# nirajbabar/raytracinginonesemester

Hardware: AMD Instinct MI355X
Metric: Mrays/s at 1920x1080x16spp (1/2/4/8 GPU) + PPM max-abs pixel diff (higher is better)
Workload: dtype f32+f64

## Files before the change

include/rt_mi355x.h:

```cpp
#ifndef RT_MI355X_H
#define RT_MI355X_H

#include <stddef.h>
#include <stdint.h>

#ifdef __cplusplus
extern "C" {
#endif

#define RT_ABI_VERSION 3

enum {
    RT_OK = 0,
    RT_ERR_ARG = -1,
    RT_ERR_IO = -2,
    RT_ERR_PARSE = -3,
    RT_ERR_HIP = -4,
    RT_ERR_NOMEM = -5,
    RT_ERR_NODEVICE = -6,
    RT_ERR_UNSUPPORTED = -7,
    RT_ERR_COMM = -8,
    RT_ERR_INTERNAL = -9
};

// ... 408 lines not shown
int rt_heavy_tiles(const rt_scene* s, int64_t* heavy);
const char* rt_scene_kernel_name(const rt_scene* s);

int rt_scene_traversal_info(const rt_scene* s, int64_t info[4]);
int rt_scene_faults(rt_scene* s, uint32_t* flags, int clear);

typedef enum {
    RT_TUNE_FRUSTUM_ARITY = 0,
    RT_TUNE_HALF_WAVES = 1,
    RT_TUNE_PAIRED_ONLY = 2,
    RT_TUNE_HEAVY_FRAC = 3,
    RT_TUNE_HEAVY_CAP = 4,
    RT_TUNE_CULL_COVERAGE = 5,
    RT_TUNE_CULL_BOXES = 6,
    RT_TUNE_BIG_SCENE_BYTES = 7,
    RT_TUNE_FRUSTUM_STACK_CAP = 8,
    RT_TUNE_PEER_TIMEOUT_S = 9,
    RT_TUNE_RENDERER_THREADS = 10,
    RT_TUNE_COPY_ENGINE = 11,
    RT_TUNE_QUANT_RECORDS = 12,
    RT_TUNE_PREPASS_GATE = 13,
    RT_TUNE_OVERLAP_FRAMES = 14,
    RT_TUNE_KERNEL_TIMING_EVERY = 15,
    RT_TUNE_RECORD_GREEDY = 16,
    RT_TUNE_WIDE4_GREEDY = 17,
    RT_TUNE_PAIR_FRAMES = 18,
    RT_TUNE_PAIR_RESERVE = 19,
    RT_TUNE_CUT_SUB = 20,
    RT_TUNE_HW1_LANES = 21,
    RT_TUNE_COPY_WAIT = 22,
    RT_TUNE_HW1_FUSE = 23,
    RT_TUNE_HW1_CHUNK = 24,
    RT_TUNE_FRAME_STREAMS = 25,
    RT_TUNE_COUNT = 26
} rt_tune_id;
int rt_tuning_set(int id, double value);
int rt_tuning_get(int id, double* value);
void rt_tuning_reset(void);

int rt_device_count(int* n);
const char* rt_last_error(void);
int rt_abi_version(void);
const char* rt_build_id(void);

#ifdef __cplusplus
}
#endif
#endif
```

raytracinginonesemester_amd/_lib.py:

```python
from __future__ import annotations

import ctypes as C
import os
from pathlib import Path

PKG = Path(__file__).resolve().parent
LIB_PATH = Path(os.environ.get("RT_MI355X_LIB", PKG / "lib" / "librt_mi355x.so"))

RT_OK = 0
RT_ERR = {
    -1: "RT_ERR_ARG", -2: "RT_ERR_IO", -3: "RT_ERR_PARSE", -4: "RT_ERR_HIP",
    -5: "RT_ERR_NOMEM", -6: "RT_ERR_NODEVICE", -7: "RT_ERR_UNSUPPORTED", -8: "RT_ERR_COMM",
    -9: "RT_ERR_INTERNAL",
}
RT_KERNEL_AUTO, RT_KERNEL_WAVE, RT_KERNEL_LANE, RT_KERNEL_WAVE_PIXELS = 0, 1, 2, 3
RT_TILES_AUTO, RT_TILES_LINEAR, RT_TILES_XCD_CHUNK, RT_TILES_ROWS = 0, 1, 2, 3
RT_FLAG_NO_CULL = 1
RT_FLAG_BINARY = 4
RT_DELIVER_P6, RT_DELIVER_F32, RT_DELIVER_DEVICE, RT_DELIVER_NONE = 0, 1, 2, 3
RT_GATHER_AUTO, RT_GATHER_RCCL, RT_GATHER_DIRECT, RT_GATHER_HOST_SHARED = 0, 1, 2, 3
RT_RENDERER_SELF_SEND = 1
RT_TIME_GATHER, RT_TIME_DELIVER, RT_TIME_FRAME = 0, 1, 2
RT_FAULT_FRUSTUM_STACK = 1
RT_RAYS_CLOSEST, RT_RAYS_OCCLUDED = 0, 1
RT_RAYS_VARIANT_NONE, RT_RAYS_VARIANT_WIDE, RT_RAYS_VARIANT_BINARY, RT_RAYS_VARIANT_DEEP = 0, 1, 2, 3
RT_REBUILD_NONE, RT_REBUILD_DEVICE, RT_REBUILD_HOST = 0, 1, 2
RT_PATH_LAST = 16
RT_PATH_NONE = 0xFFFFFFFF
RT_PIXEL_NONE = 0xFFFFFFFF
TUNE = {"frustum_arity": 0, "half_waves": 1, "paired_only": 2, "heavy_frac": 3, "heavy_cap": 4,
        "cull_coverage": 5, "cull_boxes": 6, "big_scene_bytes": 7, "frustum_stack_cap": 8,
        "peer_timeout_s": 9, "renderer_threads": 10, "copy_engine": 11,
        "quant_records": 12, "prepass_gate": 13,
        "overlap_frames": 14, "kernel_timing_every": 15,
        "record_greedy": 16, "wide4_greedy": 17, "pair_frames": 18, "pair_reserve": 19,
        "cut_sub": 20, "hw1_lanes": 21, "copy_wait": 22, "hw1_fuse": 23, "hw1_chunk": 24,
        "frame_streams": 25}


class RTError(RuntimeError):
    def __init__(self, code: int, msg: str):
        super().__init__(f"{RT_ERR.get(code, code)}: {msg}")
        self.code = code


class Vec3(C.Structure):
    _fields_ = [("x", C.c_float), ("y", C.c_float), ("z", C.c_float)]

    def __iter__(self):
        return iter((self.x, self.y, self.z))


class BVHNode(C.Structure):
    _fields_ = [("parent_idx", C.c_uint32), ("left_idx", C.c_uint32),
                ("right_idx", C.c_uint32), ("object_idx", C.c_uint32)]


class AABB(C.Structure):
    _fields_ = [("min_corner", Vec3), ("max_corner", Vec3)]


class Triangle(C.Structure):
    _fields_ = [("v0", Vec3), ("v1", Vec3), ("v2", Vec3), ("n0", Vec3), ("n1", Vec3), ("n2", Vec3)]


class Material(C.Structure):
    _fields_ = [("albedo", Vec3), ("kd", C.c_float), ("specular_color", Vec3), ("ks", C.c_float),
                ("shininess", C.c_float), ("kr", C.c_float), ("emission", Vec3)]


# ... 257 lines not shown
```

raytracinginonesemester_amd/csrc/rt_device.hip:

```cpp

#include <hip/hip_runtime.h>
#include <hip/hip_ext.h>

#include <cfloat>
#include <cmath>
#include <cstdint>
#include <cstdio>
#include <cstdlib>
#include <cstring>
#include <algorithm>
#include <atomic>
#include <functional>
#include <memory>
#include <new>
#include <string>
#include <array>
#include <vector>

#include "rt_common.hpp"
#include "rt_hip_host.hpp"
#include "rt_math.hpp"
#include "rt_ppm.hpp"
#include "rt_scene_pack.hpp"

using namespace rtd;

namespace {

using rt::LEAF_BIT;
using rt::NO_REF;
using rt::FRUSTUM_STACK;
using rt::STACK_CAP;
using rt::LANE_LDS_CAP;
using rt::kBigSceneBytes;
constexpr uint32_t RT_FAULT_FRUSTUM_STACK = 1u;
constexpr uint32_t VER_FORCE = 0xFFFFFFFFu;
constexpr int BLOCK = 256;
constexpr int MODE_WIDE = 16;
constexpr int MODE_PK = 32;
constexpr int MODE_DEEP = 64;
constexpr int MODE_1L = 128;
constexpr int MODE_QR = 256;
constexpr int REF_STACK = 512;
constexpr uint32_t INV_LEAF = 0xFFFFFFFEu;
constexpr uint32_t BRUTE_BIT = 0x40000000u;
constexpr float RT_EPS = 1e-3f;

struct DevMaterial {
    float albedo[3], kd, spec[3], ks, shininess, kr, emission[3];
};
struct DevLight {
    float pos[3], color[3];
    int32_t intensity;
};

struct SceneView {
    const float4* __restrict__ inode;
    const float4* __restrict__ wnode;
    const float* __restrict__ fnode;
    int32_t f_log2;
    const uint4* __restrict__ qent;
    const float4* __restrict__ qhdr;
    const float4* __restrict__ ibox;
    const float4* __restrict__ rootb;
    const float4* __restrict__ leaf;
    const float4* __restrict__ tnorm;
    const int32_t* __restrict__ objids;
    const DevMaterial* __restrict__ mats;
    const DevLight* __restrict__ lights;
    int32_t num_tris, num_mats, num_lights;
    uint32_t root_ref;
    float root_box[6];
    float bmax[3];
    int32_t wide;
    int32_t lane_stack;
    int32_t lane_wide;
    const float* __restrict__ cut;
    int32_t ncut;
    const float* __restrict__ cut2;
    int32_t cut_sub_log2;
    const float4* __restrict__ tri;
    uint32_t* fault;
};

__device__ __forceinline__ f3 scene_bmax(const SceneView& sc) { return mk(sc.bmax[0], sc.bmax[1], sc.bmax[2]); }

struct RenderParams {
    SceneView sc;
    f3 cam_center, cam_p00, cam_du, cam_dv;
    int32_t W, H, spp, max_depth, diffuse_bounce;
    f3 miss;
    const float* __restrict__ jitter;
    int32_t band_rows, band_index, band_count, rows;
    int32_t tile_w, tile_h, tiles_x, tiles_total;
    int32_t lane_samples;
    int32_t half_waves;
    int32_t paired_only;
    int32_t tile_order;
    int32_t spp_log2, tile_w_log2;
    int32_t cull;
    f3 miss_pixel;
    uint32_t* live_count;
    int32_t* live_tiles;
    int32_t* cut_tiles;
    uint32_t* next_count;
    int32_t cut_force;
    int32_t nqueues;
    int32_t queue_cap;
    float* __restrict__ rgb;
    int32_t* __restrict__ hit_idx;
    float* __restrict__ hit_t;
    uint8_t* __restrict__ p6;
    uint8_t miss_p6[4];
    uint16_t* __restrict__ tile_cost;
    int32_t* heavy_tiles;
    int32_t heavy_cap;
    uint32_t heavy_ticks[8];
    unsigned long long* ray_count;
    uint32_t* drained;
    uint32_t drain_tag;
    int32_t gate_q8;
};

#include "rt_wave.hpp"
#include "rt_instrument.hpp"
#include "rt_traverse.hpp"
#include "rt_shade.hpp"
#include "rt_prepass.hpp"
#include "rt_query.hpp"
#include "rt_path.hpp"
#include "rt_refit.hpp"
#include "rt_rebuild.hpp"

__device__ __forceinline__ int work_length(const RenderParams& P, int q, int& heavy) {
    heavy = 0;
    if (P.heavy_cap > 0)
        for (int k = 0; k < NCLASS; ++k) heavy += min((int)ldc_u32(P.live_count + heavy_counter(k, q)), P.heavy_cap);
    const int slot = P.sc.ncut > 0 ? CUT_SLOT0 + q : q;
    return heavy + (int)ldc_u32(&P.live_count[slot * COUNTER_STRIDE]);
}

// ... 1234 lines not shown
    hipExtLaunchKernelGGL(KERNEL, grid, dim3(BLOCK), 0, L.st, L.start, L.stop, 0, P);
}

template <int MODE, bool SAMPLES, bool D1, int WAVES = RT_RENDER_WAVES, int LS = 0>
void launch_render_pair(const RenderParams& A, const RenderParams& B, const Launch& L, double reserve_default) {
    constexpr auto KERNEL = render_pair_kernel<MODE, SAMPLES, D1, WAVES, LS>;
    static const int per_cu = [] {
        int n = 0;
        if (hipOccupancyMaxActiveBlocksPerMultiprocessor(&n, KERNEL, BLOCK, 0) != hipSuccess || n < 1) n = 1;
        return n;
    }();
    static const std::string name = "render_pair_kernel<" + std::to_string(MODE) + (SAMPLES ? ", true" : ", false") +
                                    (D1 ? ", true, " : ", false, ") + std::to_string(WAVES) + ", " +
                                    std::to_string(LS) + ">";
    if (L.name) *L.name = name.c_str();
    const int tiles8 = (A.tiles_total + B.tiles_total + 7) / 8 * 8;
    const double reserve = std::clamp(rt::tuning(RT_TUNE_PAIR_RESERVE, reserve_default), 0.0, double(per_cu - 1));
    const int blocks = L.cus * per_cu - int(std::lround(reserve * L.cus));
    const dim3 grid((unsigned)std::max(8, std::min(tiles8, blocks / 8 * 8)));
    PairParams PP;
    PP.f[0] = A;
    PP.f[1] = B;
    hipExtLaunchKernelGGL(KERNEL, grid, dim3(BLOCK), 0, L.st, L.start, L.stop, 0, PP);
}

bool pair_kernel_fits(const RenderParams& P, bool samples, bool wave_wide, bool big) {
    const bool d1 = P.max_depth == 1;
    const bool bounce = P.max_depth > 1 && P.half_waves && P.paired_only;
    return samples && wave_wide && !big && (d1 || bounce) && P.nqueues == 8 && P.spp <= 64 && !P.ray_count &&
           P.lane_samples == 1;
}
void launch_pair(const RenderParams& A, const RenderParams& B, const Launch& L) {
    constexpr int M = RT_KERNEL_WAVE | MODE_WIDE | MODE_PK;
    if (A.max_depth > 1) launch_render_pair<RT_KERNEL_WAVE | MODE_WIDE, true, false, RT_PAIRED_WAVES, 3>(A, B, L, 0.0);
    else if (A.half_waves) launch_render_pair<M, true, true, RT_RENDER_WAVES, 1>(A, B, L, 1.0);
    else launch_render_pair<M, true, true>(A, B, L, 1.0);
}

template <int MODE, bool SAMPLES>
void launch_mode(const RenderParams& P, const Launch& L) {
    constexpr int D1_MODE = (MODE & (MODE_DEEP | RT_KERNEL_LANE)) == 0 ? (MODE | MODE_PK) : MODE;
    if (P.max_depth == 1) {
        if constexpr (SAMPLES) {
            if (P.half_waves) {
                launch_render<D1_MODE, SAMPLES, true, RT_RENDER_WAVES, 1>(P, L);
                return;
            }
        }
        if constexpr ((MODE & (MODE_DEEP | RT_KERNEL_LANE)) == 0) {
            if (L.big) {
                if constexpr ((MODE & MODE_WIDE) != 0) {
                    if (L.qr) {
                        if (P.sc.num_lights == 1)
                            launch_render<D1_MODE | MODE_1L | MODE_QR, SAMPLES, true, RT_RENDER_WAVES_BIG>(P, L);
                        else launch_render<D1_MODE | MODE_QR, SAMPLES, true, RT_RENDER_WAVES_BIG>(P, L);
                        return;
                    }
                }
                if (P.sc.num_lights == 1) launch_render<D1_MODE | MODE_1L, SAMPLES, true, RT_RENDER_WAVES_BIG>(P, L);
                else launch_render<D1_MODE, SAMPLES, true, RT_RENDER_WAVES_BIG>(P, L);
                return;
            }
        }
        launch_render<D1_MODE, SAMPLES, true>(P, L);
    } else {
        if constexpr (SAMPLES && (MODE & (MODE_DEEP | RT_KERNEL_LANE)) == 0) {
            if (P.half_waves && P.paired_only) {
                launch_render<MODE, SAMPLES, false, RT_PAIRED_WAVES, 3>(P, L);
                return;
            }
        }
        if constexpr (SAMPLES) {
            if (P.half_waves) {
                launch_render<MODE, SAMPLES, false, RT_BOUNCE_WAVES, 1>(P, L);
                return;
            }
        }
        launch_render<MODE, SAMPLES, false, RT_BOUNCE_WAVES>(P, L);
    }
}

template <int MODE>
void launch(const RenderParams& P, bool samples, const Launch& L) {
    if (samples) launch_mode<MODE, true>(P, L);
    else launch_mode<MODE, false>(P, L);
}

f3 miss_pixel_value(const rt_render_opts* o) {
    f3 c = mk(0.f, 0.f, 0.f);
    if (o->max_depth > 0)
        c = clamp01(add(mk(0.f, 0.f, 0.f), mul(mk(1.f, 1.f, 1.f), f3{o->miss_color.x, o->miss_color.y, o->miss_color.z})));
    f3 acc = mk(0.f, 0.f, 0.f);
    for (int k = 0; k < o->spp; ++k) acc = add(acc, c);
    const float fs = (float)o->spp;
    return f3{acc.x / fs, acc.y / fs, acc.z / fs};
}

// ... 139 lines not shown
    P.hit_idx = hit_idx;
    P.hit_t = hit_t;
    P.p6 = p6;
    P.ray_count = t_ray_count;
    {
        const f3 mp = miss_pixel_value(o);
        P.miss_p6[0] = rtp::p6_default_sample(mp.x);
        P.miss_p6[1] = rtp::p6_default_sample(mp.y);
        P.miss_p6[2] = rtp::p6_default_sample(mp.z);
        P.miss_p6[3] = 0;
    }
    const bool samples = o->kernel != RT_KERNEL_WAVE_PIXELS && o->spp <= BLOCK && (o->spp & (o->spp - 1)) == 0;
    int half = o->band_count >= 4 || o->max_depth > 1 ? 1 : 0;
    if (const double h = rt::tuning(RT_TUNE_HALF_WAVES, -1.0); h >= 0.0) half = h >= 1.0 ? 1 : 0;
    if (!samples || o->spp > (64 >> half)) half = 0;
    P.half_waves = half;
    P.paired_only = half && o->max_depth > 1 && s->nlights == 1 && !s->deep && o->kernel != RT_KERNEL_LANE &&
                            (P.sc.wide ? s->lane_wide : s->lane_stack)
                        ? 1
                        : 0;
    P.paired_only = P.paired_only && rt::tuning(RT_TUNE_PAIRED_ONLY, 1.0) != 0.0;
    int ppb = samples ? (BLOCK >> half) / o->spp : BLOCK;
    int tw = 1;
    while (tw * tw < ppb) tw <<= 1;
    int th = ppb / tw;
    P.tile_w = tw;
    P.tile_h = th;
    P.tile_w_log2 = __builtin_ctz(unsigned(tw));
    P.spp_log2 = samples ? __builtin_ctz(unsigned(o->spp)) : 0;
    P.tiles_x = (W + tw - 1) / tw;
    const int tiles_y = (rows + th - 1) / th;
    P.tiles_total = P.tiles_x * tiles_y;
    P.lane_samples = samples ? 1 : 0;
    P.tile_order = o->tile_order == RT_TILES_AUTO ? RT_TILES_ROWS : o->tile_order;
    P.cull = (o->flags & RT_FLAG_NO_CULL) ? 0 : 1;
    if (!P.cull) P.sc.ncut = 0;
    P.miss_pixel = miss_pixel_value(o);
    P.nqueues = P.tile_order == RT_TILES_LINEAR ? 1 : 8;
    P.queue_cap = P.tile_order == RT_TILES_LINEAR ? P.tiles_total : P.tiles_x * ((tiles_y + 7) / 8);
    const double heavy_frac = rt::tuning(RT_TUNE_HEAVY_FRAC, 0.10);
    const int mode = o->kernel == RT_KERNEL_LANE ? RT_KERNEL_LANE : RT_KERNEL_WAVE;
    const bool costs = P.cull && P.sc.ncut > 0 && P.nqueues == 8 && heavy_frac > 0.0;
    const int heavy_cap = int(std::clamp(rt::tuning(RT_TUNE_HEAVY_CAP, 512.0), 1.0, 1e9));
    P.heavy_cap = costs ? std::min(P.queue_cap, heavy_cap) : 0;
    constexpr size_t kCounterBytes = COUNTER_SET_U32 * sizeof(uint32_t);
    const size_t list_bytes = size_t(P.nqueues) * size_t(P.queue_cap) * sizeof(int32_t);
    const size_t cut_bytes = P.sc.ncut > 0 ? list_bytes : 0;
    const size_t heavy_bytes = size_t(8 * NCLASS) * size_t(P.heavy_cap) * sizeof(int32_t);
    const size_t set_bytes = list_bytes + cut_bytes + heavy_bytes;
    const size_t work_bytes = rt_scene::kSets * (kCounterBytes + set_bytes);
    hipStream_t st = static_cast<hipStream_t>(stream);
    const uint64_t k = s->launches;
    auto ev1_of = [&](uint64_t f) { return s->ev1[f % rt_scene::kRing]; };
    bool pair_b = ps && ps->phase == 1 && ps->deferred;
    if (pair_b) {
        const RenderParams& A = ps->A;
        const bool same = A.tiles_total == P.tiles_total && A.tiles_x == P.tiles_x && A.W == P.W && A.rows == P.rows &&
                          A.spp == P.spp && A.half_waves == P.half_waves && A.sc.ncut == P.sc.ncut && A.cull == P.cull &&
                          A.heavy_cap == P.heavy_cap && A.queue_cap == P.queue_cap && A.nqueues == P.nqueues &&
                          A.max_depth == P.max_depth && A.paired_only == P.paired_only && A.band_index == P.band_index &&
                          A.band_count == P.band_count && ps->stream == static_cast<hipStream_t>(stream);
        if (!same) {
            pair_b = false;
            if ((rc = flush_pair_a(s, *ps)) != RT_OK) return rc;
        }
    }
// ... 1086 lines not shown
```

raytracinginonesemester_amd/csrc/rt_shade.hpp:

```cpp
#pragma once

template <bool DEEP = false>
__device__ __forceinline__ int32_t leaf_tri(const SceneView& sc, int32_t slot) {
    if constexpr (DEEP) {
        if ((uint32_t)slot & BRUTE_BIT) return (int32_t)((uint32_t)slot & ~BRUTE_BIT);
    }
    return __float_as_int(sc.leaf[4 * (size_t)slot].w);
}

struct SurfHit {
    f3 p, n;
    int32_t tri;
};

template <bool DEEP = false>
__device__ __forceinline__ SurfHit resolve_hit(const SceneView& sc, const RayPre& r, int32_t slot) {
    const float4* L = sc.leaf + 4 * (size_t)slot;
    bool brute = false;
    if constexpr (DEEP) {
        brute = ((uint32_t)slot & BRUTE_BIT) != 0;
        if (brute) L = sc.tri + 3 * (size_t)((uint32_t)slot & ~BRUTE_BIT);
    }
    const float4 a = L[0], b = L[1], c = L[2];
    const f3 v0 = mk(a.x, a.y, a.z), e1 = mk(b.x, b.y, b.z), e2 = mk(b.w, c.x, c.y);
// ... 88 lines not shown
            const SurfHit sh = resolve_hit<(MODE & MODE_DEEP) != 0>(sc, cray, slot);
            const f3 N = unit(sh.n);
            const f3 V = unit(sub(cray.o, sh.p));
            const f3 L = unit(sub(lpos, sh.p));
            const float NdotL = fmaxf(dot(N, L), 0.0f);
            if (NdotL > 0.0f) {
                const DevMaterial m = material_of(sc, sh.tri);
                const f3 f = eval_brdf(m, sh.n, V, L);
                const f3 rad = scale(mk(lt.color[0], lt.color[1], lt.color[2]), (float)lt.intensity);
                Lo_lit = add(Lo, scale(mul(rad, f), NdotL));
                lit = true;
                const f3 toL = sub(lpos, sh.p);
                dist = sqrtf(dot(toL, toL));
                if (dist > 0.0f) {
                    need = true;
                    sray = make_ray(add(sh.p, scale(N, RT_EPS)), divf(toL, dist), scene_bmax(sc));
                }
            }
        }
        pk.put(0, cray.d.x);
        pk.put(1, cray.d.y);
        pk.put(2, cray.d.z);
        pk.put(3, __int_as_float(slot));
        pk.put(4, Lo.x);
        pk.put(5, Lo.y);
        pk.put(6, Lo.z);
        pk.put(7, Lo_lit.x);
        pk.put(8, Lo_lit.y);
        pk.put(9, Lo_lit.z);
        pk.put(11, lit ? 1.0f : 0.0f);
        Park::fence();
        HitState shs;
        count_rays<MODE>(P.ray_count, 1, need);
        traverse<MODE>(sc, sray, need, true, dist, shs);
        const bool occluded = need && shs.slot >= 0 && shs.bestT < dist;
        Park::fence();
        const int fl = __float_as_int(pk.get(10));
        valid = (fl & 1) != 0;
        hit = (fl & 2) != 0;
        lit = pk.get(11) != 0.0f;
        const bool take = lit && !occluded;
        Lo = take ? mk(pk.get(7), pk.get(8), pk.get(9)) : mk(pk.get(4), pk.get(5), pk.get(6));
        slot = __float_as_int(pk.get(3));
        cray.d = mk(pk.get(0), pk.get(1), pk.get(2));
    };
    if ((MODE & MODE_1L) != 0) {
        light(0);
    } else if (sc.num_lights == 1) {
        light(0);
    } else {
        for (int li = 0; li < sc.num_lights; ++li) light(li);
    }
    return radiance_of(Lo);
}


#ifndef RT_NO_RESUME
#define RT_RESUME 1
#endif
#ifdef RT_RESUME
#ifndef RT_RESUME_SHIFT
#define RT_RESUME_SHIFT 2
#endif
struct LaneDfs {
    uint32_t ref;
    int sp, stale;
    bool retest, run;
// ... 461 lines not shown
```

raytracinginonesemester_amd/csrc/rt_traverse.hpp:

```cpp
#pragma once

__device__ __forceinline__ v2f lo2(float4 q) { return (v2f){q.x, q.y}; }
__device__ __forceinline__ v2f hi2(float4 q) { return (v2f){q.z, q.w}; }

__device__ __forceinline__ BoxP own_box(const SceneView& sc, uint32_t ref, bool is_root) {
    BoxP b;
    if (is_root) {
        const float4 p = ldc(sc.rootb), q = ldc(sc.rootb + 1);
        b.x = lo2(p);
        b.y = hi2(p);
        b.z = lo2(q);
    } else if (ref & LEAF_BIT) {
        const float4* L = sc.leaf + 4 * (size_t)(ref & ~LEAF_BIT);
        const float4 c = ldc(L + 2), d = ldc(L + 3);
        b.x = hi2(c);
        b.y = lo2(d);
        b.z = hi2(d);
    } else {
        const float4* B = sc.ibox + 2 * (size_t)ref;
        const float4 p = ldc(B), q = ldc(B + 1);
        b.x = lo2(p);
        b.y = hi2(p);
        b.z = lo2(q);
    }
// ... 164 lines not shown
                        }
                    }
                }
            }
        }
        if (pmask != 0) {
            ref = pref;
            mask = pmask;
        } else {
            if (sp == 0) break;
            --sp;
            ref = rdlane(st_ref, sp);
            mask = ((uint64_t)rdlane(st_mhi, sp) << 32) | rdlane(st_mlo, sp);
            if (any_hit) mask &= alive;
            if (sp < stale) {
                stale = sp;
                RT_STAT(6 + so, 1);
                BoxP ob;
                if (ref & LEAF_BIT) {
                    const float4* L = reinterpret_cast<const float4*>(leaf_b + ((ref & ~LEAF_BIT) << 6));
                    const float4 c = ldc(L + 2), d = ldc(L + 3);
                    ob = BoxP{hi2(c), lo2(d), hi2(d)};
                } else {
                    const float4* B = reinterpret_cast<const float4*>(ibox_b + (ref << 5));
                    const float4 p = ldc(B), q = ldc(B + 1);
                    ob = BoxP{lo2(p), hi2(p), lo2(q)};
                }
                mask = box_hit_mask<PK, XL>(r, ob, hs.bestT, mask);
            }
        }
    }
}

__device__ __forceinline__ bool family_dirs(const SceneView& sc, const RayPre& r, bool member, const float* o, v2f* U) {
    const float dd[3] = {r.d.x, r.d.y, r.d.z};
    bool loose = false;
#pragma unroll
    for (int a = 0; a < 3; ++a) {
        const float dl = wave_reduce_f<false>(member ? dd[a] : INFINITY);
        const float dh = wave_reduce_f<true>(member ? dd[a] : -INFINITY);
        const bool fin = sc.bmax[a] + fabsf(o[a]) < 1e30f;
        const bool ok = (dl >= 1e-8f || dh <= -1e-8f) && fin;
        const bool lz = !ok && fin;
        loose = loose || lz;
        const float u0 = ok ? rcp_approx(dl) : lz ? (dh > 0.0f ? rcp_approx(dh) : INFINITY) : -INFINITY;
        const float u1 = ok ? rcp_approx(dh) : lz ? (dl < 0.0f ? rcp_approx(dl) : -INFINITY) : INFINITY;
        U[a] = (v2f){__int_as_float(uni(__float_as_int(u0))), __int_as_float(uni(__float_as_int(u1)))};
    }
    return loose;
}

template <bool PK, bool XL, bool QR, bool LOOSE>
__device__ __forceinline__ void frustum_loop(const SceneView& sc, const RayPre& r, bool live, HitState& hs,
                                             const float* o, const v2f* U);
template <bool PK = false, bool XL = false, bool QR = false>
__device__ __forceinline__ void traverse_frustum(const SceneView& sc, const RayPre& r, bool active, HitState& hs) {
    hs.bestT = FLT_MAX;
    hs.slot = -1;
#ifdef RT_STATS
    hs.pops = 0;
#endif
    uint64_t alive = ballot(active);
    if (alive == 0) return;
    RT_STAT(0, 1);
    RT_STAT(13, __popcll(alive));
    alive = box_hit_mask<PK, XL>(r, own_box(sc, sc.root_ref, true), FLT_MAX, alive);
    if (alive == 0) {
        RT_STAT(17, 1);
        return;
    }
    const bool live = lane_in(alive);
    const float o[3] = {__int_as_float(uni(__float_as_int(r.o.x))), __int_as_float(uni(__float_as_int(r.o.y))),
                        __int_as_float(uni(__float_as_int(r.o.z)))};
    v2f U[3];
    const bool loose = family_dirs(sc, r, live, o, U);
    if (__builtin_amdgcn_readfirstlane((int)loose) != 0) frustum_loop<PK, XL, QR, true>(sc, r, live, hs, o, U);
    else frustum_loop<PK, XL, QR, false>(sc, r, live, hs, o, U);
}

template <bool PK, bool XL, bool QR, bool LOOSE>
__device__ __forceinline__ void frustum_loop(const SceneView& sc, const RayPre& r, bool live, HitState& hs,
                                             const float* o, const v2f* U) {
    const float kW = 1.0f / 524288.0f;
    float tmax_w = FLT_MAX;
    uint32_t ref = sc.root_ref;
    uint32_t st_ref = 0, st_hi = 0;
    int sp = 0;
    bool ovf = false;
    const char* leaf_b = reinterpret_cast<const char*>(sc.leaf);
    const uint32_t lg = (uint32_t)sc.f_log2;
    const char* rec_b = sc.fnode != nullptr ? reinterpret_cast<const char*>(sc.fnode) : reinterpret_cast<const char*>(sc.wnode);
    const uint32_t rec_shift = 5u + lg;
    const uint32_t ent_mask = (uint32_t)((1ull << (1u << lg)) - 1ull);
    const uint32_t kl = fresh_lane_id() & ((1u << lg) - 1u);
    const uint32_t k6 = 6u * kl, kref = (6u << lg) + kl;
    while (true) {
        RT_STAT(2, 1);
#ifdef RT_STATS
        ++hs.pops;
#endif
        uint32_t next = NO_REF;
        if (ref & LEAF_BIT) {
            RT_STAT(10, 1);
            const uint32_t slot = ref & ~LEAF_BIT;
            const float4* L = reinterpret_cast<const float4*>(leaf_b + (slot << 6));
            const float4 a = ldc(L), b = ldc(L + 1), c = ldc(L + 2), d = ldc(L + 3);
            float t, u, v;
            const bool hm = live && mt_g(r, mk(a.x, a.y, a.z), mk(b.x, b.y, b.z), mk(b.w, c.x, c.y),
                                                  kRayTMin, hs.bestT, t, u, v);
            const uint64_t mh = ballot(hm);
            if (mh != 0) {
                RT_STAT(4, 1);
                const uint64_t m = box_hit_mask<PK, XL>(r, BoxP{hi2(c), lo2(d), hi2(d)}, hs.bestT, mh);
                if (m != 0) {
                    if (lane_in(m)) {
                        hs.bestT = t;
                        hs.slot = (int32_t)slot;
                    }
                    tmax_w = wave_reduce_f<true>(live ? hs.bestT : 0.0f);
                }
            }
        } else {
            RT_STAT(8, 1);
            v2f bb[3];
            uint32_t rk;
            if constexpr (QR) {
                const vf4 g0 = ldc_v(sc.qhdr + 2 * ref), g1 = ldc_v(sc.qhdr + 2 * ref + 1);
                const uint4 e = sc.qent[((size_t)ref << lg) + kl];
                const float og[3] = {g0.x, g0.y, g0.z}, st[3] = {g0.w, g1.x, g1.y};
                const uint32_t qw[3] = {e.x, e.y, e.z};
#pragma unroll
                for (int a = 0; a < 3; ++a) {
                    const v2f q = {(float)(qw[a] & 0xFFFFu), (float)(qw[a] >> 16)};
                    bb[a] = __builtin_elementwise_fma(q, (v2f){st[a], st[a]}, (v2f){og[a], og[a]});
                }
                rk = e.w;
            } else {
                const float* W = reinterpret_cast<const float*>(rec_b + ((size_t)ref << rec_shift));
                const v2f* B = reinterpret_cast<const v2f*>(W + k6);
                bb[0] = B[0];
                bb[1] = B[1];
                bb[2] = B[2];
                rk = reinterpret_cast<const uint32_t*>(W)[kref];
            }
            float nr[3], fr[3];
#pragma unroll
            for (int a = 0; a < 3; ++a) {
                const v2f db = bb[a] - (v2f){o[a], o[a]};
                const v2f p = (v2f){db.x, db.x} * U[a], q = (v2f){db.y, db.y} * U[a];
                nr[a] = fminf(fminf(p.x, p.y), fminf(q.x, q.y));
                fr[a] = fmaxf(fmaxf(p.x, p.y), fmaxf(q.x, q.y));
                if constexpr (LOOSE) {
                    if (U[a].x > 0.0f && U[a].y < 0.0f) {
                        nr[a] = fmaxf(p.x, q.y);
                        fr[a] = INFINITY;
                    }
                }
            }
            float Lc = fmaxf(fmaxf(nr[0], nr[1]), nr[2]);
            float Hc = fminf(fminf(fr[0], fr[1]), fr[2]);
            Lc = __builtin_fmaf(fabsf(Lc), -kW, Lc);
            Hc = __builtin_fmaf(fabsf(Hc), kW, Hc);
            const uint32_t m =
                (uint32_t)ballot(rk != NO_REF && fmaxf(Lc, kRayTMin) <= fminf(Hc, tmax_w)) & ent_mask;
            if (m != 0) {
                RT_STAT(4, 1);
                const uint32_t hold = 31u - __builtin_clz(m);
                next = rdlane(rk, hold);
                for (uint32_t rest = m & ~(1u << hold); rest != 0; rest &= rest - 1u) {
                    const uint32_t e = rdlane(rk, __builtin_ctz(rest));
                    if (sp < 64) {
                        st_ref = wrlane(e, sp, st_ref);
                    } else if (sp < FRUSTUM_STACK) {
                        st_hi = wrlane(e, sp - 64, st_hi);
                    } else {
                        ovf = true;
                        continue;
                    }
                    ++sp;
                }
            }
        }
        if (next != NO_REF) {
            ref = next;
            continue;
        }
        if (sp == 0) break;
        --sp;
        ref = sp < 64 ? rdlane(st_ref, sp) : rdlane(st_hi, sp - 64);
    }
    if (ovf) {
        if (fresh_lane_id() == 0) atomicOr(sc.fault, RT_FAULT_FRUSTUM_STACK);
        hs.bestT = __int_as_float(0x7fc00000);
        hs.slot = -1;
    }
}

__device__ __forceinline__ void traverse_lane(const SceneView& sc, const RayPre& r, bool active,
                                              bool any_hit, float any_hit_dist, HitState& hs) {
// ... 224 lines not shown
template <bool WIDE>
__device__ __forceinline__ void traverse_lane(const SceneView& sc, const RayPre& r, bool active, bool any_hit,
                                              float any_hit_dist, HitState& hs, uint32_t* stk) {
    if constexpr (WIDE) traverse_lane_lds_wide(sc, r, active, any_hit, any_hit_dist, hs, stk);
    else traverse_lane_lds(sc, r, active, any_hit, any_hit_dist, hs, stk);
}
template <bool WIDE>
__device__ __forceinline__ bool lane_ok(const SceneView& sc) {
    return WIDE ? sc.lane_wide != 0 : sc.lane_stack != 0;
}

template <int MODE>
__device__ __forceinline__ void traverse(const SceneView& sc, const RayPre& r, bool active, bool any_hit,
                                         float any_hit_dist, HitState& hs) {
    if constexpr ((MODE & MODE_DEEP) != 0) traverse_deep(sc, r, active, any_hit, any_hit_dist, hs);
    else if constexpr (MODE == RT_KERNEL_LANE) traverse_lane(sc, r, active, any_hit, any_hit_dist, hs);
    else traverse_wave_split<(MODE & MODE_WIDE) != 0, (MODE & MODE_PK) != 0, (MODE & MODE_PK) != 0 && (MODE & MODE_1L) == 0>(
        sc, r, active, any_hit, any_hit_dist, hs);
}

template <int MODE>
__device__ __forceinline__ void traverse_camera(const SceneView& sc, const RayPre& r, bool active, HitState& hs) {
#ifndef RT_NO_FRUSTUM
    if constexpr (MODE != RT_KERNEL_LANE && (MODE & MODE_DEEP) == 0 && (MODE & MODE_WIDE) != 0) {
        traverse_frustum<(MODE & MODE_PK) != 0, (MODE & MODE_PK) != 0 && (MODE & MODE_1L) == 0, (MODE & MODE_QR) != 0>(
            sc, r, active, hs);
        return;
    }
#endif
    traverse<MODE>(sc, r, active, false, 0.0f, hs);
}

template <int MODE>
__device__ __forceinline__ void traverse_at(const SceneView& sc, int depth, const RayPre& r, bool active, bool any_hit,
                                            float any_hit_dist, HitState& hs, float* lds) {
    if constexpr (MODE != RT_KERNEL_LANE && (MODE & MODE_DEEP) == 0) {
        constexpr bool W = (MODE & MODE_WIDE) != 0;
        if (depth > 0 && lane_ok<W>(sc)) {
            traverse_lane<W>(sc, r, active, any_hit, any_hit_dist, hs, reinterpret_cast<uint32_t*>(lds));
#ifdef RT_LANE_ITERS
            lane_iters_note(active ? hs.iters : 0u);
#endif
            return;
        }
    }
    traverse<MODE>(sc, r, active, any_hit, any_hit_dist, hs);
}
```

Before: 247,400.

## Add wave-coherent frustum traversal for shadow rays on big single-light scenes

Adds a shadow-ray path that builds a wave-wide frustum from the per-lane origin bounds and direction bounds. Whole BVH nodes are culled against that frustum, and traversal exits early once every lane is occluded. The path is gated by an origin-spread heuristic scaled by pixel footprint, and is enabled by default only for big scenes with one light that are not in half-wave mode. It targets incoherent per-ray shadow traversal, at the cost of extra template variants, more register pressure, and a fallback when the frustum is loose or too wide.

```diff
diff --git a/include/rt_mi355x.h b/include/rt_mi355x.h
--- a/include/rt_mi355x.h
+++ b/include/rt_mi355x.h
@@ -464,7 +464,8 @@
     RT_TUNE_HW1_FUSE = 23,
     RT_TUNE_HW1_CHUNK = 24,
     RT_TUNE_FRAME_STREAMS = 25,
-    RT_TUNE_COUNT = 26
+    RT_TUNE_SHADOW_FRUSTUM = 26,
+    RT_TUNE_COUNT = 27
 } rt_tune_id;
 int rt_tuning_set(int id, double value);
 int rt_tuning_get(int id, double* value);
diff --git a/raytracinginonesemester_amd/_lib.py b/raytracinginonesemester_amd/_lib.py
--- a/raytracinginonesemester_amd/_lib.py
+++ b/raytracinginonesemester_amd/_lib.py
@@ -35,7 +35,7 @@
         "overlap_frames": 14, "kernel_timing_every": 15,
         "record_greedy": 16, "wide4_greedy": 17, "pair_frames": 18, "pair_reserve": 19,
         "cut_sub": 20, "hw1_lanes": 21, "copy_wait": 22, "hw1_fuse": 23, "hw1_chunk": 24,
-        "frame_streams": 25}
+        "frame_streams": 25, "shadow_frustum": 26}
 
 
 class RTError(RuntimeError):
diff --git a/raytracinginonesemester_amd/csrc/rt_device.hip b/raytracinginonesemester_amd/csrc/rt_device.hip
--- a/raytracinginonesemester_amd/csrc/rt_device.hip
+++ b/raytracinginonesemester_amd/csrc/rt_device.hip
@@ -20,6 +20,7 @@
 #include "rt_common.hpp"
 #include "rt_hip_host.hpp"
 #include "rt_math.hpp"
+#include "rt_family.hpp"
 #include "rt_ppm.hpp"
 #include "rt_scene_pack.hpp"
 
@@ -41,10 +42,16 @@
 constexpr int MODE_DEEP = 64;
 constexpr int MODE_1L = 128;
 constexpr int MODE_QR = 256;
+constexpr int MODE_SF = 512;
+constexpr bool shadow_frustum_kernel(int mode) {
+    return (mode & MODE_DEEP) == 0 && (mode & MODE_WIDE) != 0 && (mode & RT_KERNEL_WAVE) != 0 &&
+           (mode & (MODE_SF | MODE_1L)) != 0;
+}
 constexpr int REF_STACK = 512;
 constexpr uint32_t INV_LEAF = 0xFFFFFFFEu;
 constexpr uint32_t BRUTE_BIT = 0x40000000u;
 constexpr float RT_EPS = 1e-3f;
+constexpr double kShadowFrustumBigK = 8.0;
 
 struct DevMaterial {
     float albedo[3], kd, spec[3], ks, shininess, kr, emission[3];
@@ -107,6 +114,7 @@
     int32_t cut_force;
     int32_t nqueues;
     int32_t queue_cap;
+    float shadow_kw;
     float* __restrict__ rgb;
     int32_t* __restrict__ hit_idx;
     float* __restrict__ hit_t;
@@ -1407,9 +1415,23 @@
 }
 void launch_pair(const RenderParams& A, const RenderParams& B, const Launch& L) {
     constexpr int M = RT_KERNEL_WAVE | MODE_WIDE | MODE_PK;
+    const bool sf = A.shadow_kw > 0.0f;
     if (A.max_depth > 1) launch_render_pair<RT_KERNEL_WAVE | MODE_WIDE, true, false, RT_PAIRED_WAVES, 3>(A, B, L, 0.0);
+    else if (A.half_waves && sf) launch_render_pair<M | MODE_SF, true, true, RT_RENDER_WAVES, 1>(A, B, L, 1.0);
     else if (A.half_waves) launch_render_pair<M, true, true, RT_RENDER_WAVES, 1>(A, B, L, 1.0);
+    else if (sf) launch_render_pair<M | MODE_SF, true, true>(A, B, L, 1.0);
     else launch_render_pair<M, true, true>(A, B, L, 1.0);
+}
+
+template <int MODE, bool SAMPLES, int WAVES = RT_RENDER_WAVES, int LS = 0>
+void launch_d1(const RenderParams& P, const Launch& L) {
+    if constexpr ((MODE & (MODE_DEEP | RT_KERNEL_LANE)) == 0 && (MODE & MODE_WIDE) != 0 && !shadow_frustum_kernel(MODE)) {
+        if (P.shadow_kw > 0.0f) {
+            launch_render<MODE | MODE_SF, SAMPLES, true, WAVES, LS>(P, L);
+            return;
+        }
+    }
+    launch_render<MODE, SAMPLES, true, WAVES, LS>(P, L);
 }
 
 template <int MODE, bool SAMPLES>
@@ -1418,7 +1440,7 @@
     if (P.max_depth == 1) {
         if constexpr (SAMPLES) {
             if (P.half_waves) {
-                launch_render<D1_MODE, SAMPLES, true, RT_RENDER_WAVES, 1>(P, L);
+                launch_d1<D1_MODE, SAMPLES, RT_RENDER_WAVES, 1>(P, L);
                 return;
             }
         }
@@ -1426,18 +1448,17 @@
             if (L.big) {
                 if constexpr ((MODE & MODE_WIDE) != 0) {
                     if (L.qr) {
-                        if (P.sc.num_lights == 1)
-                            launch_render<D1_MODE | MODE_1L | MODE_QR, SAMPLES, true, RT_RENDER_WAVES_BIG>(P, L);
-                        else launch_render<D1_MODE | MODE_QR, SAMPLES, true, RT_RENDER_WAVES_BIG>(P, L);
+                        if (P.sc.num_lights == 1) launch_d1<D1_MODE | MODE_1L | MODE_QR, SAMPLES, RT_RENDER_WAVES_BIG>(P, L);
+                        else launch_d1<D1_MODE | MODE_QR, SAMPLES, RT_RENDER_WAVES_BIG>(P, L);
                         return;
                     }
                 }
-                if (P.sc.num_lights == 1) launch_render<D1_MODE | MODE_1L, SAMPLES, true, RT_RENDER_WAVES_BIG>(P, L);
-                else launch_render<D1_MODE, SAMPLES, true, RT_RENDER_WAVES_BIG>(P, L);
+                if (P.sc.num_lights == 1) launch_d1<D1_MODE | MODE_1L, SAMPLES, RT_RENDER_WAVES_BIG>(P, L);
+                else launch_d1<D1_MODE, SAMPLES, RT_RENDER_WAVES_BIG>(P, L);
                 return;
             }
         }
-        launch_render<D1_MODE, SAMPLES, true>(P, L);
+        launch_d1<D1_MODE, SAMPLES>(P, L);
     } else {
         if constexpr (SAMPLES && (MODE & (MODE_DEEP | RT_KERNEL_LANE)) == 0) {
             if (P.half_waves && P.paired_only) {
@@ -1643,6 +1664,19 @@
     const int tiles_y = (rows + th - 1) / th;
     P.tiles_total = P.tiles_x * tiles_y;
     P.lane_samples = samples ? 1 : 0;
+    {
+        const bool big_scene =
+            !half && s->nlights == 1 &&
+            double(s->bytes) > std::max(0.0, rt::tuning(RT_TUNE_BIG_SCENE_BYTES, double(kBigSceneBytes)));
+        const double k = rt::tuning(RT_TUNE_SHADOW_FRUSTUM, big_scene ? kShadowFrustumBigK : 0.0);
+        const double side = std::sqrt(double(samples ? std::max(1, (64 >> half) / o->spp) : 64)) + 1.0;
+        const f3 mid = add(add(P.cam_p00, scale(P.cam_du, 0.5f * float(W))), scale(P.cam_dv, 0.5f * float(H)));
+        const f3 ax = sub(mid, P.cam_center);
+        const double focal = std::sqrt(double(dot(ax, ax)));
+        const double pix = std::sqrt(double(std::max(dot(P.cam_du, P.cam_du), dot(P.cam_dv, P.cam_dv))));
+        const double kw = k * side * pix / focal;
+        P.shadow_kw = !(k > 0.0) ? 0.0f : (k >= 1e30 || !(kw < 1e30)) ? INFINITY : float(kw);
+    }
     P.tile_order = o->tile_order == RT_TILES_AUTO ? RT_TILES_ROWS : o->tile_order;
     P.cull = (o->flags & RT_FLAG_NO_CULL) ? 0 : 1;
     if (!P.cull) P.sc.ncut = 0;
diff --git a/raytracinginonesemester_amd/csrc/rt_family.hpp b/raytracinginonesemester_amd/csrc/rt_family.hpp
--- /dev/null
+++ b/raytracinginonesemester_amd/csrc/rt_family.hpp
@@ -0,0 +1,62 @@
+#pragma once
+
+#include <cfloat>
+#include <cmath>
+
+#if defined(__HIPCC__)
+#define RT_FAMILY_HD __host__ __device__ __forceinline__
+#else
+#define RT_FAMILY_HD inline
+#endif
+
+#if defined(__clang__)
+typedef float fam_v2 __attribute__((ext_vector_type(2)));
+#else
+typedef float fam_v2 __attribute__((vector_size(8)));
+#endif
+
+constexpr float kFamilyTMin = 1e-4f;
+constexpr float kFamilyWiden = 1.0f / 524288.0f;
+
+RT_FAMILY_HD float family_rcp(float x) {
+#if defined(__HIP_DEVICE_COMPILE__)
+    return __builtin_amdgcn_rcpf(x);
+#else
+    return 1.0f / x;
+#endif
+}
+
+RT_FAMILY_HD bool family_axis(float dl, float dh, float ol, float oh, float bmax, fam_v2& U) {
+    const bool fin = bmax + fmaxf(fabsf(ol), fabsf(oh)) < 1e30f;
+    const bool ok = (dl >= 1e-8f || dh <= -1e-8f) && fin;
+    const bool lz = !ok && fin;
+    const float u0 = ok ? family_rcp(dl) : lz ? (dh > 0.0f ? family_rcp(dh) : INFINITY) : -INFINITY;
+    const float u1 = ok ? family_rcp(dh) : lz ? (dl < 0.0f ? family_rcp(dl) : -INFINITY) : INFINITY;
+    U = (fam_v2){u0, u1};
+    return lz;
+}
+
+template <bool LOOSE>
+RT_FAMILY_HD bool family_entry_pass(const fam_v2* bb, const float* oh, const float* ol, const fam_v2* U, float tmax_w) {
+    float nr[3], fr[3];
+#if defined(__clang__)
+#pragma unroll
+#endif
+    for (int a = 0; a < 3; ++a) {
+        const fam_v2 db = bb[a] - (fam_v2){oh[a], ol[a]};
+        const fam_v2 p = (fam_v2){db[0], db[0]} * U[a], q = (fam_v2){db[1], db[1]} * U[a];
+        nr[a] = fminf(fminf(p[0], p[1]), fminf(q[0], q[1]));
+        fr[a] = fmaxf(fmaxf(p[0], p[1]), fmaxf(q[0], q[1]));
+        if (LOOSE) {
+            if (U[a][0] > 0.0f && U[a][1] < 0.0f) {
+                nr[a] = fmaxf(p[0], q[1]);
+                fr[a] = INFINITY;
+            }
+        }
+    }
+    float Lc = fmaxf(fmaxf(nr[0], nr[1]), nr[2]);
+    float Hc = fminf(fminf(fr[0], fr[1]), fr[2]);
+    Lc = __builtin_fmaf(fabsf(Lc), -kFamilyWiden, Lc);
+    Hc = __builtin_fmaf(fabsf(Hc), kFamilyWiden, Hc);
+    return fmaxf(Lc, kFamilyTMin) <= fminf(Hc, tmax_w);
+}
diff --git a/raytracinginonesemester_amd/csrc/rt_shade.hpp b/raytracinginonesemester_amd/csrc/rt_shade.hpp
--- a/raytracinginonesemester_amd/csrc/rt_shade.hpp
+++ b/raytracinginonesemester_amd/csrc/rt_shade.hpp
@@ -144,7 +144,8 @@
         Park::fence();
         HitState shs;
         count_rays<MODE>(P.ray_count, 1, need);
-        traverse<MODE>(sc, sray, need, true, dist, shs);
+        if constexpr (shadow_frustum_kernel(MODE)) traverse_shadow<MODE>(P, sray, need, dist, shs);
+        else traverse<MODE>(sc, sray, need, true, dist, shs);
         const bool occluded = need && shs.slot >= 0 && shs.bestT < dist;
         Park::fence();
         const int fl = __float_as_int(pk.get(10));
diff --git a/raytracinginonesemester_amd/csrc/rt_traverse.hpp b/raytracinginonesemester_amd/csrc/rt_traverse.hpp
--- a/raytracinginonesemester_amd/csrc/rt_traverse.hpp
+++ b/raytracinginonesemester_amd/csrc/rt_traverse.hpp
@@ -220,27 +220,25 @@
     }
 }
 
-__device__ __forceinline__ bool family_dirs(const SceneView& sc, const RayPre& r, bool member, const float* o, v2f* U) {
+__device__ __forceinline__ bool family_dirs(const SceneView& sc, const RayPre& r, bool member, const float* oh,
+                                            const float* ol, v2f* U) {
     const float dd[3] = {r.d.x, r.d.y, r.d.z};
     bool loose = false;
 #pragma unroll
     for (int a = 0; a < 3; ++a) {
         const float dl = wave_reduce_f<false>(member ? dd[a] : INFINITY);
         const float dh = wave_reduce_f<true>(member ? dd[a] : -INFINITY);
-        const bool fin = sc.bmax[a] + fabsf(o[a]) < 1e30f;
-        const bool ok = (dl >= 1e-8f || dh <= -1e-8f) && fin;
-        const bool lz = !ok && fin;
+        v2f u;
+        const bool lz = family_axis(dl, dh, ol[a], oh[a], sc.bmax[a], u);
         loose = loose || lz;
-        const float u0 = ok ? rcp_approx(dl) : lz ? (dh > 0.0f ? rcp_approx(dh) : INFINITY) : -INFINITY;
-        const float u1 = ok ? rcp_approx(dh) : lz ? (dl < 0.0f ? rcp_approx(dl) : -INFINITY) : INFINITY;
-        U[a] = (v2f){__int_as_float(uni(__float_as_int(u0))), __int_as_float(uni(__float_as_int(u1)))};
+        U[a] = (v2f){__int_as_float(uni(__float_as_int(u.x))), __int_as_float(uni(__float_as_int(u.y)))};
     }
     return loose;
 }
 
-template <bool PK, bool XL, bool QR, bool LOOSE>
+template <bool PK, bool XL, bool QR, bool LOOSE, bool SHADOW = false>
 __device__ __forceinline__ void frustum_loop(const SceneView& sc, const RayPre& r, bool live, HitState& hs,
-                                             const float* o, const v2f* U);
+                                             const float* oh, const float* ol, const v2f* U, float dist = 0.0f);
 template <bool PK = false, bool XL = false, bool QR = false>
 __device__ __forceinline__ void traverse_frustum(const SceneView& sc, const RayPre& r, bool active, HitState& hs) {
     hs.bestT = FLT_MAX;
@@ -261,15 +259,60 @@
     const float o[3] = {__int_as_float(uni(__float_as_int(r.o.x))), __int_as_float(uni(__float_as_int(r.o.y))),
                         __int_as_float(uni(__float_as_int(r.o.z)))};
     v2f U[3];
-    const bool loose = family_dirs(sc, r, live, o, U);
-    if (__builtin_amdgcn_readfirstlane((int)loose) != 0) frustum_loop<PK, XL, QR, true>(sc, r, live, hs, o, U);
-    else frustum_loop<PK, XL, QR, false>(sc, r, live, hs, o, U);
-}
-
-template <bool PK, bool XL, bool QR, bool LOOSE>
-__device__ __forceinline__ void frustum_loop(const SceneView& sc, const RayPre& r, bool live, HitState& hs,
-                                             const float* o, const v2f* U) {
-    const float kW = 1.0f / 524288.0f;
+    const bool loose = family_dirs(sc, r, live, o, o, U);
+    if (__builtin_amdgcn_readfirstlane((int)loose) != 0) frustum_loop<PK, XL, QR, true>(sc, r, live, hs, o, o, U);
+    else frustum_loop<PK, XL, QR, false>(sc, r, live, hs, o, o, U);
+}
+
+template <bool PK = false, bool XL = false, bool QR = false>
+__device__ __forceinline__ bool traverse_frustum_shadow(const SceneView& sc, const RayPre& r, bool need, float dist,
+                                                        f3 cam, float kw, HitState& hs) {
+    hs.bestT = FLT_MAX;
+    hs.slot = -1;
+#ifdef RT_STATS
+    hs.pops = 0;
+#endif
+    uint64_t alive = ballot(need);
+    if (alive == 0) return true;
+    alive = box_hit_mask<PK, XL>(r, own_box(sc, sc.root_ref, true), FLT_MAX, alive);
+    if (alive == 0) {
+        RT_STAT(1, 1);
+        RT_STAT(14, __popcll(ballot(need)));
+        return true;
+    }
+    const bool live = lane_in(alive);
+    const float oo[3] = {r.o.x, r.o.y, r.o.z};
+    float oh[3], ol[3];
+    float ext = 0.0f;
+#pragma unroll
+    for (int a = 0; a < 3; ++a) {
+        ol[a] = __int_as_float(uni(__float_as_int(wave_reduce_f<false>(live ? oo[a] : INFINITY))));
+        oh[a] = __int_as_float(uni(__float_as_int(wave_reduce_f<true>(live ? oo[a] : -INFINITY))));
+        ext = fmaxf(ext, oh[a] - ol[a]);
+    }
+    const f3 oc = sub(r.o, cam);
+    const float far = kw * sqrtf(wave_reduce_f<true>(live ? dot(oc, oc) : 0.0f));
+    if (__builtin_amdgcn_readfirstlane((int)!(ext <= far)) != 0) {
+        RT_STAT(22, 1);
+        return false;
+    }
+    v2f U[3];
+    const bool loose = family_dirs(sc, r, live, oh, ol, U);
+    if (__builtin_amdgcn_readfirstlane((int)loose) != 0) {
+        RT_STAT(21, 1);
+        return false;
+    }
+    RT_STAT(1, 1);
+    RT_STAT(14, __popcll(ballot(need)));
+    RT_STAT(20, 1);
+    frustum_loop<PK, XL, QR, false, true>(sc, r, live, hs, oh, ol, U, dist);
+    return true;
+}
+
+template <bool PK, bool XL, bool QR, bool LOOSE, bool SHADOW>
+__device__ __forceinline__ void frustum_loop(const SceneView& sc, const RayPre& r, bool live_in, HitState& hs,
+                                             const float* oh, const float* ol, const v2f* U, float dist) {
+    bool live = live_in;
     float tmax_w = FLT_MAX;
     uint32_t ref = sc.root_ref;
     uint32_t st_ref = 0, st_hi = 0;
@@ -280,16 +323,21 @@
     const char* rec_b = sc.fnode != nullptr ? reinterpret_cast<const char*>(sc.fnode) : reinterpret_cast<const char*>(sc.wnode);
     const uint32_t rec_shift = 5u + lg;
     const uint32_t ent_mask = (uint32_t)((1ull << (1u << lg)) - 1ull);
-    const uint32_t kl = fresh_lane_id() & ((1u << lg) - 1u);
-    const uint32_t k6 = 6u * kl, kref = (6u << lg) + kl;
+    uint32_t kl = 0, k6 = 0, kref = 0;
+    auto entry_lane = [&] {
+        kl = fresh_lane_id() & ((1u << lg) - 1u);
+        k6 = 6u * kl;
+        kref = (6u << lg) + kl;
+    };
+    if constexpr (!SHADOW) entry_lane();
     while (true) {
-        RT_STAT(2, 1);
+        RT_STAT(2 + SHADOW, 1);
 #ifdef RT_STATS
         ++hs.pops;
 #endif
         uint32_t next = NO_REF;
         if (ref & LEAF_BIT) {
-            RT_STAT(10, 1);
+            RT_STAT(10 + SHADOW, 1);
             const uint32_t slot = ref & ~LEAF_BIT;
             const float4* L = reinterpret_cast<const float4*>(leaf_b + (slot << 6));
             const float4 a = ldc(L), b = ldc(L + 1), c = ldc(L + 2), d = ldc(L + 3);
@@ -298,18 +346,23 @@
                                                   kRayTMin, hs.bestT, t, u, v);
             const uint64_t mh = ballot(hm);
             if (mh != 0) {
-                RT_STAT(4, 1);
+                RT_STAT(4 + SHADOW, 1);
                 const uint64_t m = box_hit_mask<PK, XL>(r, BoxP{hi2(c), lo2(d), hi2(d)}, hs.bestT, mh);
                 if (m != 0) {
                     if (lane_in(m)) {
                         hs.bestT = t;
                         hs.slot = (int32_t)slot;
                     }
+                    if constexpr (SHADOW) {
+                        live = live && !(hs.bestT < dist);
+                        if (ballot(live) == 0) break;
+                    }
                     tmax_w = wave_reduce_f<true>(live ? hs.bestT : 0.0f);
                 }
             }
         } else {
-            RT_STAT(8, 1);
+            RT_STAT(8 + SHADOW, 1);
+            if constexpr (SHADOW) entry_lane();
             v2f bb[3];
             uint32_t rk;
             if constexpr (QR) {
@@ -331,28 +384,10 @@
                 bb[2] = B[2];
                 rk = reinterpret_cast<const uint32_t*>(W)[kref];
             }
-            float nr[3], fr[3];
-#pragma unroll
-            for (int a = 0; a < 3; ++a) {
-                const v2f db = bb[a] - (v2f){o[a], o[a]};
-                const v2f p = (v2f){db.x, db.x} * U[a], q = (v2f){db.y, db.y} * U[a];
-                nr[a] = fminf(fminf(p.x, p.y), fminf(q.x, q.y));
-                fr[a] = fmaxf(fmaxf(p.x, p.y), fmaxf(q.x, q.y));
-                if constexpr (LOOSE) {
-                    if (U[a].x > 0.0f && U[a].y < 0.0f) {
-                        nr[a] = fmaxf(p.x, q.y);
-                        fr[a] = INFINITY;
-                    }
-                }
-            }
-            float Lc = fmaxf(fmaxf(nr[0], nr[1]), nr[2]);
-            float Hc = fminf(fminf(fr[0], fr[1]), fr[2]);
-            Lc = __builtin_fmaf(fabsf(Lc), -kW, Lc);
-            Hc = __builtin_fmaf(fabsf(Hc), kW, Hc);
             const uint32_t m =
-                (uint32_t)ballot(rk != NO_REF && fmaxf(Lc, kRayTMin) <= fminf(Hc, tmax_w)) & ent_mask;
+                (uint32_t)ballot(rk != NO_REF && family_entry_pass<LOOSE>(bb, oh, ol, U, tmax_w)) & ent_mask;
             if (m != 0) {
-                RT_STAT(4, 1);
+                RT_STAT(4 + SHADOW, 1);
                 const uint32_t hold = 31u - __builtin_clz(m);
                 next = rdlane(rk, hold);
                 for (uint32_t rest = m & ~(1u << hold); rest != 0; rest &= rest - 1u) {
@@ -643,6 +678,20 @@
 }
 
 template <int MODE>
+__device__ __forceinline__ void traverse_shadow(const RenderParams& P, const RayPre& r, bool need, float dist,
+                                                HitState& hs) {
+#ifndef RT_NO_FRUSTUM
+    if constexpr (shadow_frustum_kernel(MODE)) {
+        if (P.shadow_kw > 0.0f &&
+            traverse_frustum_shadow<(MODE & MODE_PK) != 0, (MODE & MODE_PK) != 0 && (MODE & MODE_1L) == 0,
+                                    (MODE & MODE_QR) != 0>(P.sc, r, need, dist, P.cam_center, P.shadow_kw, hs))
+            return;
+    }
+#endif
+    traverse<MODE>(P.sc, r, need, true, dist, hs);
+}
+
+template <int MODE>
 __device__ __forceinline__ void traverse_at(const SceneView& sc, int depth, const RayPre& r, bool active, bool any_hit,
                                             float any_hit_dist, HitState& hs, float* lds) {
     if constexpr (MODE != RT_KERNEL_LANE && (MODE & MODE_DEEP) == 0) {
```

Result: slower. 244,100 (-1.3%).
